# AlgoLab/rs-vgaligner

Hardware: AMD Instinct MI355X
Metric: aligned reads/sec (10 kbp ONT vs HLA graph) (higher is better)
Workload: dtype int32+f64

## Files before the change

### rs-vgaligner_amd/csrc/vga_poa_row.hpp

```cpp
#pragma once

#include "vga_poa_launch.hpp"
#include "vga_poa_kernels.hpp"

#define T4_NEG (4 * POA_NEG)

template <int B>
__device__ __forceinline__ int t4_sub_byte(int a, int g)
{
    int r;
    if constexpr (B == 0) asm("v_sub_u32_sdwa %0, %1, %2 dst_sel:DWORD dst_unused:UNUSED_PAD src0_sel:DWORD src1_sel:BYTE_0" : "=v"(r) : "v"(a), "v"(g));
    if constexpr (B == 1) asm("v_sub_u32_sdwa %0, %1, %2 dst_sel:DWORD dst_unused:UNUSED_PAD src0_sel:DWORD src1_sel:BYTE_1" : "=v"(r) : "v"(a), "v"(g));
    if constexpr (B == 2) asm("v_sub_u32_sdwa %0, %1, %2 dst_sel:DWORD dst_unused:UNUSED_PAD src0_sel:DWORD src1_sel:BYTE_2" : "=v"(r) : "v"(a), "v"(g));
    if constexpr (B == 3) asm("v_sub_u32_sdwa %0, %1, %2 dst_sel:DWORD dst_unused:UNUSED_PAD src0_sel:DWORD src1_sel:BYTE_3" : "=v"(r) : "v"(a), "v"(g));
    return r;
}
template <int B>
__device__ __forceinline__ void t4_gap_byte(int &dst, int &acc, int t, int c)
{
    if constexpr (B == 0) asm("v_min_u32_sdwa %0, %2, %3 dst_sel:BYTE_0 dst_unused:UNUSED_PRESERVE src0_sel:DWORD src1_sel:DWORD\n\tv_cmp_le_u32 vcc, %3, %2\n\tv_addc_co_u32 %1, vcc, %1, %1, vcc" : "+v"(dst), "+v"(acc) : "v"(t), "s"(c) : "vcc");
    if constexpr (B == 1) asm("v_min_u32_sdwa %0, %2, %3 dst_sel:BYTE_1 dst_unused:UNUSED_PRESERVE src0_sel:DWORD src1_sel:DWORD\n\tv_cmp_le_u32 vcc, %3, %2\n\tv_addc_co_u32 %1, vcc, %1, %1, vcc" : "+v"(dst), "+v"(acc) : "v"(t), "s"(c) : "vcc");
    if constexpr (B == 2) asm("v_min_u32_sdwa %0, %2, %3 dst_sel:BYTE_2 dst_unused:UNUSED_PRESERVE src0_sel:DWORD src1_sel:DWORD\n\tv_cmp_le_u32 vcc, %3, %2\n\tv_addc_co_u32 %1, vcc, %1, %1, vcc" : "+v"(dst), "+v"(acc) : "v"(t), "s"(c) : "vcc");
    if constexpr (B == 3) asm("v_min_u32_sdwa %0, %2, %3 dst_sel:BYTE_3 dst_unused:UNUSED_PRESERVE src0_sel:DWORD src1_sel:DWORD\n\tv_cmp_le_u32 vcc, %3, %2\n\tv_addc_co_u32 %1, vcc, %1, %1, vcc" : "+v"(dst), "+v"(acc) : "v"(t), "s"(c) : "vcc");
}
__device__ __forceinline__ void t4_flag_ne(int &acc, int a, int b)
{
    asm("v_cmp_ne_u32 vcc, %1, %2\n\tv_addc_co_u32 %0, vcc, %0, %0, vcc" : "+v"(acc) : "v"(a), "v"(b) : "vcc");
}
template <int B>
__device__ __forceinline__ void t4_flag_ne_dep(int &dst, int acc, int a, int b)
{
    if constexpr (B == 0) asm("v_cmp_ne_u32 vcc, %2, %3\n\tv_addc_co_u32_sdwa %0, vcc, %1, %1, vcc dst_sel:BYTE_0 dst_unused:UNUSED_PRESERVE src0_sel:DWORD src1_sel:DWORD" : "+v"(dst) : "v"(acc), "v"(a), "v"(b) : "vcc");
    if constexpr (B == 1) asm("v_cmp_ne_u32 vcc, %2, %3\n\tv_addc_co_u32_sdwa %0, vcc, %1, %1, vcc dst_sel:BYTE_1 dst_unused:UNUSED_PRESERVE src0_sel:DWORD src1_sel:DWORD" : "+v"(dst) : "v"(acc), "v"(a), "v"(b) : "vcc");
    if constexpr (B == 2) asm("v_cmp_ne_u32 vcc, %2, %3\n\tv_addc_co_u32_sdwa %0, vcc, %1, %1, vcc dst_sel:BYTE_2 dst_unused:UNUSED_PRESERVE src0_sel:DWORD src1_sel:DWORD" : "+v"(dst) : "v"(acc), "v"(a), "v"(b) : "vcc");
    if constexpr (B == 3) asm("v_cmp_ne_u32 vcc, %2, %3\n\tv_addc_co_u32_sdwa %0, vcc, %1, %1, vcc dst_sel:BYTE_3 dst_unused:UNUSED_PRESERVE src0_sel:DWORD src1_sel:DWORD" : "+v"(dst) : "v"(acc), "v"(a), "v"(b) : "vcc");
}
__device__ __forceinline__ int t4_max3(int a, int b, int c)
{
    int r;
    asm("v_max3_i32 %0, %1, %2, %3" : "=v"(r) : "v"(a), "v"(b), "v"(c));
    return r;
}
__device__ __forceinline__ int t4_shr1_max(int v, int pre)
{
    int r = pre;
    asm("s_nop 1\n\tv_max_i32_dpp %0, %1, %2 wave_shr:1 row_mask:0xf bank_mask:0xf" : "+v"(r) : "v"(v), "v"(pre));
    return r;
}
__device__ __forceinline__ int t4_shr1_mov(int v, int first)
{
    int r = first;
    asm("s_nop 1\n\tv_mov_b32_dpp %0, %1 wave_shr:1 row_mask:0xf bank_mask:0xf" : "+v"(r) : "v"(v));
    return r;
}

template <int B>
__device__ __forceinline__ void t5_min_byte(int &dst, int t, int c)
{
    if constexpr (B == 0) asm("v_min_u32_sdwa %0, %1, %2 dst_sel:BYTE_0 dst_unused:UNUSED_PRESERVE src0_sel:DWORD src1_sel:DWORD" : "+v"(dst) : "v"(t), "s"(c));
    if constexpr (B == 1) asm("v_min_u32_sdwa %0, %1, %2 dst_sel:BYTE_1 dst_unused:UNUSED_PRESERVE src0_sel:DWORD src1_sel:DWORD" : "+v"(dst) : "v"(t), "s"(c));
    if constexpr (B == 2) asm("v_min_u32_sdwa %0, %1, %2 dst_sel:BYTE_2 dst_unused:UNUSED_PRESERVE src0_sel:DWORD src1_sel:DWORD" : "+v"(dst) : "v"(t), "s"(c));
    if constexpr (B == 3) asm("v_min_u32_sdwa %0, %1, %2 dst_sel:BYTE_3 dst_unused:UNUSED_PRESERVE src0_sel:DWORD src1_sel:DWORD" : "+v"(dst) : "v"(t), "s"(c));
}

__device__ __forceinline__ int t5_own(int v)
{
    asm volatile("" : "+v"(v));
    return __builtin_amdgcn_readfirstlane(v);
}
__device__ __forceinline__ uint32_t t5_own(uint32_t v) { return (uint32_t)t5_own((int)v); }
__device__ __forceinline__ uint64_t t5_own(uint64_t v) { return ((uint64_t)t5_own((uint32_t)(v >> 32)) << 32) | t5_own((uint32_t)v); }
template <typename T>
__device__ __forceinline__ T *t5_own(T *p) { return (T *)t5_own((uint64_t)p); }


struct poa_row_view {
    int qlen;
    const char *query;
    const uint4 *ntab;
    const uint32_t *plist, *seqw;
    poa_row *R;
    uint32_t n_nodes, ring_rows;
    int bw, banded, p_match, p_mismatch;
};
__device__ __forceinline__ poa_row_view poa_row_view_of(const poa_prob &pb, const char *queries, const uint4 *node_tab, const uint32_t *seq32,
                                                        const uint32_t *preds, const poa_t5_args &A)
{
    poa_row_view V;
    V.qlen = t5_own((int)pb.qlen);
    V.query = queries + pb.q0;
    V.ntab = node_tab + t5_own(pb.node0);
    V.plist = preds + t5_own(pb.pred0);
    V.seqw = seq32 + t5_own(pb.seq0 >> 2);
    V.R = A.rows + t5_own(pb.row0);
    V.n_nodes = t5_own(pb.n_nodes);
    V.ring_rows = t5_own(pb.ring_rows);
    V.bw = t5_own((int)pb.w);
    V.banded = t5_own(A.P.banded);
    V.p_match = t5_own(A.P.match);
    V.p_mismatch = t5_own(A.P.mismatch);
    return V;
}
struct poa_row_pen {
    int o1, e1, o2, e2, D1, D2;
    uint32_t g_bias, e_probe;
};
template <bool DEF>
__device__ __forceinline__ poa_row_pen poa_row_pen_of(const poa_dev_params &P)
{
    poa_row_pen K;
    K.o1 = DEF ? 4 : t5_own(P.o1); K.e1 = DEF ? 2 : t5_own(P.e1); K.o2 = DEF ? 24 : t5_own(P.o2); K.e2 = DEF ? 1 : t5_own(P.e2);
    K.D1 = 4 * K.o1; K.D2 = 4 * K.o2 + 1;
    K.g_bias = (uint32_t)(4 * K.e1 | (4 * K.e2) << 8) * 0x00010001u;
    K.e_probe = (uint32_t)((128 - K.D1) | (128 - K.D2) << 8) * 0x00010001u;
    return K;
}

__device__ __forceinline__ bool poa_row_state(const poa_t5_args &A, int got, bool first_thread, uint64_t &state_lo)
{
    if (got < 0) {
        if (first_thread) {
            poa_out &O = A.outs[blockIdx.x];
            O.t_end = O.t_begin; O.cells = 0; O.vcells = 0; O.maxw = 0; O.nops = 0;
            O.score = POA_NEG; O.row = 0; O.status = A.cp.n_slots ? POA_ST_POOL : POA_ST_RETRY;
        }
        return false;
    }
    __builtin_amdgcn_fence(__ATOMIC_ACQUIRE, "agent");
    state_lo = (uint64_t)A.cp.state_base + (uint64_t)(uint32_t)got * A.cp.state_size;
    return true;
}

struct poa_chunks {
    uint32_t own_head, own_tail, own_chunks;
    uint64_t dcur;
    uint32_t drem;
};
__device__ __forceinline__ uint32_t poa_chunks_pop(const poa_chunk_pool &cp, const poa_chunks &C)
{
    const uint32_t idx = poa_chunk_pop(cp, blockIdx.x);
    if (idx != POA_NIL) __hip_atomic_store(cp.next + idx, C.own_head, __ATOMIC_RELAXED, __HIP_MEMORY_SCOPE_AGENT);
    return idx;
}
__device__ __forceinline__ void poa_chunks_took(poa_chunks &C, uint32_t idx, uint64_t addr)
{
    C.own_head = idx;
    if (C.own_tail == POA_NIL) C.own_tail = idx;
    C.own_chunks++;
    C.dcur = addr;
    C.drem = (uint32_t)POA_CHUNK;
}
__device__ __forceinline__ uint64_t poa_chunks_bump(poa_chunks &C, uint32_t bytes)
{
    const uint64_t r = C.dcur;
    C.dcur += bytes;
    C.drem -= bytes;
    return r;
}

__device__ __forceinline__ int poa_row_codes(uint16_t *Qn, const char *query, int qlen, int n_hw, int tid, int nt)
{
    int non_acgt = 0;
    for (int t = tid; t < n_hw; t += nt) {
        uint32_t hw = 0;
#pragma unroll
        for (int k = 0; k < 4; k++) {
            const int j = 4 * t + k;
            uint32_t code = 0;
            if (j >= 1 && j <= qlen) {
                const char ch = query[j - 1];
                code = (ch == 'A' || ch == 'C' || ch == 'G' || ch == 'T') ? 1u << (((uint32_t)ch >> 1) & 3u) : 0u;
                non_acgt |= code == 0;
            }
            hw |= code << (4 * k);
        }
        Qn[t] = (uint16_t)hw;
    }
    return non_acgt;
}

struct poa_row_topo {
    uint32_t r;
    bool last;
    bool is_sink;
    uint32_t ps;
    uint32_t gb;
    bool simple;
    bool first;
    int np;
    int remain;
};
__device__ __forceinline__ poa_row_topo poa_row_topo_of(const uint4 nt, uint32_t v, uint32_t tn, const uint32_t *seqw, uint32_t &seq_word,
                                                        uint32_t &seq_word_idx)
{
    const uint32_t nlen = nt.y & 0xFFFFFFu;
    const int np_node = (int)(nt.y >> 24);
    poa_row_topo T;
    T.r = nt.x + tn;
    T.last = tn + 1 == nlen;
    T.is_sink = T.last && (nt.z >> 31) != 0;
    T.ps = nt.w;
    T.gb = 0;
    if (v > 0) {
        const uint32_t bi = T.r - 1;
        if ((bi & 3u) == 0 || (bi >> 2) != seq_word_idx) { seq_word_idx = bi >> 2; seq_word = seqw[seq_word_idx]; }
        T.gb = (seq_word >> (8u * (bi & 3u))) & 0xffu;
    }
    T.simple = T.r > 0 && (tn > 0 || (np_node == 1 && T.ps == T.r - 1));
    T.first = tn == 0 && v > 0;
    T.np = v == 0 ? 0 : (tn == 0 ? np_node : 1);
    T.remain = (int)(nt.z & 0x3fffffffu) + (int)(nlen - 1 - tn);
    return T;
}

__device__ __forceinline__ void poa_row_far_span(const poa_row_view &V, const poa_row_topo &T, int prev_lmax, int prev_rmax, int &mpl, int &mpr)
// ... 295 lines not shown
```

### rs-vgaligner_amd/csrc/vga_poa_t5.hpp

```cpp
#pragma once

#include "vga_poa_row.hpp"

__device__ __forceinline__ uint64_t t5_uniform64(uint64_t v)
{
    return ((uint64_t)(uint32_t)__builtin_amdgcn_readfirstlane((int)(v >> 32)) << 32) | (uint32_t)__builtin_amdgcn_readfirstlane((int)(uint32_t)v);
}

#define POA_T5_ARGS_OFFSET 40
__device__ __forceinline__ const poa_t5_args *t5_kargs()
{
    uint32_t off = POA_T5_ARGS_OFFSET;
    asm volatile("" : "+s"(off));
    return (const poa_t5_args *)((const char *)__builtin_amdgcn_kernarg_segment_ptr() + off);
}
template <int NT, bool DEF>
__global__ __launch_bounds__(NT) __attribute__((amdgpu_waves_per_eu(5)))
void k_poa_dp_t5(const poa_prob *__restrict__ probs, const char *__restrict__ queries,
                                                       const uint4 *__restrict__ node_tab, const uint32_t *__restrict__ seq32,
                                                       const uint32_t *__restrict__ preds, const poa_t5_args A)
{
    poa_row *rows = A.rows;
    uint8_t *pool_arg = A.pool;
    const uint32_t lds_cols = t5_own(A.lds_cols), hg_cols = t5_own(A.hg_cols), win_mask = t5_own(A.win_mask);
// ... 144 lines not shown
        }
    }
    if (tid == 0) { sSink[2] = POA_NEG; sSink[3] = 0; }
    int prev_beg = 0, prev_end = -1;
    uint32_t seq_word = 0, seq_word_idx = 0xFFFFFFFFu;

    for (uint32_t v = 0; v < n_nodes && !failed; v++) {
    const uint4 nt = ntab[v];
    const uint32_t nlen = nt.y & 0xFFFFFFu;
    for (uint32_t tn = 0; tn < nlen && !failed; tn++) {
        asm volatile("" : "+s"(st));
        POA_MARK("row_topo");
        const uint32_t r = nt.x + tn;
        const bool last = tn + 1 == nlen;
        const bool is_sink = last && (nt.z >> 31) != 0;
        const uint32_t ps = nt.w;
        uint32_t gb = 0;
        if (v > 0) {
            const uint32_t bi = r - 1;
            if ((bi & 3u) == 0 || (bi >> 2) != seq_word_idx) { seq_word_idx = bi >> 2; seq_word = seqw[seq_word_idx]; }
            gb = (seq_word >> (8u * (bi & 3u))) & 0xffu;
        }
        const bool simple = r > 0 && prev_lds && (tn > 0 || ((nt.y >> 24) == 1u && ps == r - 1));
        const bool writer = wv == (int)(r % (uint32_t)NW);
        POA_MARK("row_prevmax");
        int prev_lmax = 0, prev_rmax = 0;
        if (r > 0) {
            int4 rw = make_int4(INT32_MIN, INT32_MAX, INT32_MIN, 0);
            if (lane < NW) rw = sRed[lane];
            int b = rw.x, t;
            t = poa_dpp<0x111, 0xf>(INT32_MIN, b); b = t > b ? t : b;
            if (NW > 2) { t = poa_dpp<0x112, 0xf>(INT32_MIN, b); b = t > b ? t : b; }
            if (NW > 4) { t = poa_dpp<0x114, 0xf>(INT32_MIN, b); b = t > b ? t : b; }
            if (NW > 8) { t = poa_dpp<0x118, 0xf>(INT32_MIN, b); b = t > b ? t : b; }
            const int rbest = __builtin_amdgcn_readlane(b, NW - 1);
            const uint64_t tie = __builtin_amdgcn_ballot_w64(rw.x == rbest);
            if (__builtin_expect(__builtin_popcountll(tie) == 1, 1)) {
                const int w1 = __builtin_ctzll(tie);
                prev_lmax = __builtin_amdgcn_readlane(rw.y, w1);
                prev_rmax = __builtin_amdgcn_readlane(rw.z, w1);
            } else {
                int lm = rw.x == rbest ? rw.y : INT32_MAX, rm = rw.x == rbest ? rw.z : INT32_MIN;
                t = poa_dpp<0x111, 0xf>(INT32_MAX, lm); lm = t < lm ? t : lm;
                t = poa_dpp<0x111, 0xf>(INT32_MIN, rm); rm = t > rm ? t : rm;
                if (NW > 2) {
                    t = poa_dpp<0x112, 0xf>(INT32_MAX, lm); lm = t < lm ? t : lm;
                    t = poa_dpp<0x112, 0xf>(INT32_MIN, rm); rm = t > rm ? t : rm;
                }
                if (NW > 4) {
                    t = poa_dpp<0x114, 0xf>(INT32_MAX, lm); lm = t < lm ? t : lm;
                    t = poa_dpp<0x114, 0xf>(INT32_MIN, rm); rm = t > rm ? t : rm;
                }
                if (NW > 8) {
                    t = poa_dpp<0x118, 0xf>(INT32_MAX, lm); lm = t < lm ? t : lm;
                    t = poa_dpp<0x118, 0xf>(INT32_MIN, rm); rm = t > rm ? t : rm;
                }
                prev_lmax = __builtin_amdgcn_readlane(lm, NW - 1);
                prev_rmax = __builtin_amdgcn_readlane(rm, NW - 1);
            }
            if (prev_far_use && writer && lane == 0) { R[r - 1].lmax = prev_lmax; R[r - 1].rmax = prev_rmax; }
        }
        POA_MARK("row_setup");
        const int remain = (int)(nt.z & 0x3fffffffu) + (int)(nlen - 1 - tn);
        int beg, end, np, pbeg = prev_beg, pend = prev_end;
        bool first, single, sp_near;
        uint32_t sp = r - 1;
        uint64_t vpo = 0;
        if (__builtin_expect(simple, 1)) {
            first = tn == 0;
            np = 1; single = true; sp_near = true;
            const int mpl = prev_lmax + 1, mpr = prev_rmax + 1;
            if (!P.banded) { beg = 0; end = qlen; }
            else {
                const int diag = qlen - remain;
                const int lo = mpl < diag ? mpl : diag;
                const int hi = mpr > diag ? mpr : diag;
                beg = lo - bw; if (beg < 0) beg = 0;
                end = hi + bw; if (end > qlen) end = qlen;
            }
        } else {
            first = tn == 0 && v > 0;
            np = v == 0 ? 0 : (tn == 0 ? (int)(nt.y >> 24) : 1);
            bool far = r > 0 && !prev_lds;
            if (first) {
                if (np == 1) far |= ps != r - 1;
                else
                    for (int t = 0; t < np; t++) far |= plist[ps + t] != r - 1;
            }
            single = r > 0 && np == 1;
            sp = first ? ps : r - 1;
            sp_near = sp == r - 1 && prev_lds;
            if (far) __syncthreads();
            int mpl, mpr;
            if (r == 0) { mpl = 0; mpr = 0; }
            else if (!first) { mpl = prev_lmax + 1; mpr = prev_rmax + 1; }
            else {
                mpl = INT32_MAX; mpr = 0;
                for (int t = 0; t < np; t++) {
                    const uint32_t p = np == 1 ? ps : plist[ps + t];
                    int lm, rm;
                    if (p == r - 1) { lm = prev_lmax + 1; rm = prev_rmax + 1; }
                    else {
                        lm = __builtin_amdgcn_readfirstlane(R[p].lmax) + 1;
                        rm = __builtin_amdgcn_readfirstlane(R[p].rmax) + 1;
                    }
                    mpl = lm < mpl ? lm : mpl;
                    mpr = rm > mpr ? rm : mpr;
                }
            }
            if (!P.banded) { beg = 0; end = qlen; }
            else {
                const int diag = qlen - remain;
                const int lo = mpl < diag ? mpl : diag;
                const int hi = mpr > diag ? mpr : diag;
                beg = lo - bw; if (beg < 0) beg = 0;
                end = hi + bw; if (end > qlen) end = qlen;
            }
            if (single && !sp_near) {
                pbeg = __builtin_amdgcn_readfirstlane(R[sp].beg);
                pend = __builtin_amdgcn_readfirstlane(R[sp].end);
                vpo = t5_uniform64(R[sp].voff);
            }
        }
        const int bal = beg & ~3;
        const int W = (end - bal + 1 + 3) & ~3;
        const bool wide = (uint32_t)W + 8u > hg_cols;
        const bool keep = last || wide;
        const uint64_t doff = alloc(dcur, dend, (uint32_t)W * (np > 1 ? 4u : 1u), 0);
        uint64_t voff = 0;
        if (last && !failed) {
            if (r == 0 || (nt.z & 0x40000000u)) voff = chunked ? alloc(dcur, dend, 6u * (uint32_t)W, 0) : alloc(vcur, vendp, 6u * (uint32_t)W, 1);
            else {
                voff = ring_base + (uint64_t)ring_head * ((6u * (uint32_t)((qlen + 8) & ~3) + 15u) & ~15u);
                ring_head = ring_head + 1 == ring_rows ? 0 : ring_head + 1;
            }
        } else if (wide) voff = wide_scratch + (r & 1u) * 6ull * lds_cols;
        if (__builtin_expect(failed, 0)) break;
        if (writer && lane == 0) {
            uint32_t *rec = (uint32_t *)(R + r);
            *(uint4 *)rec = make_uint4((uint32_t)beg, (uint32_t)end, (uint32_t)doff, (uint32_t)(doff >> 32));
            *(uint2 *)(rec + 4) = make_uint2((uint32_t)voff, (uint32_t)(voff >> 32));
            *(HIP_vector_type<uint32_t, 3> *)(rec + 8) = HIP_vector_type<uint32_t, 3>(ps, first ? (uint32_t)np : 0u, keep ? 1u : 0u);
        }
        uint8_t *Vrow = pool + voff;
        uint8_t *drow = pool + doff;
        const uint32_t gd = gb - (uint32_t)'A';
        const bool acgt = gd < 20u && ((0x80045u >> gd) & 1u);
        const int sc_eq = acgt ? P.match : 0, sc_ne = acgt ? -P.mismatch : 0;
        const int gsh = (int)((gb >> 1) & 3u);
        const int ne4t = 4 * sc_ne + 1, mm4 = 4 * (sc_eq - sc_ne);
        const bool staged = !simple && r > 0 && !wide && q_plain;
        if (staged) {
            POA_MARK("row_stage");
            if (chunked) {
                bool no_row = false;
                for (int t = 0; t < np; t++) no_row |= t5_uniform64(R[np == 1 ? sp : plist[ps + t]].voff) == 0;
                if (__builtin_expect(no_row, 0)) st |= ST_FAILED;
            }
            for (int c0 = 0; c0 < W; c0 += STEP) {
                const int c = c0 + 4 * tid;
                const int j0 = bal + c;
                if (j0 <= end && np == 1) {
                    const int bp = __builtin_amdgcn_readfirstlane(R[sp].beg), ep = __builtin_amdgcn_readfirstlane(R[sp].end);
                    const uint64_t vq_off = t5_uniform64(R[sp].voff);
                    const uint8_t *Vq = pool + vq_off;
                    const bool vq_ok = !chunked || vq_off != 0;
                    const int balq = bp & ~3;
                    const int Wq = (ep - balq + 1 + 3) & ~3;
                    const int idx = j0 - balq;
                    int4 hv = make_int4(T4_NEG, T4_NEG, T4_NEG, T4_NEG);
                    uint2 gg = make_uint2(0u, 0u);
                    if (idx >= 0 && idx < Wq && vq_ok) {
                        hv = *(const int4 *)((const int32_t *)Vq + idx);
                        gg = *(const uint2 *)(Vq + 4ll * Wq + 2ll * idx);
                    }
                    const unsigned pspan = (unsigned)(ep - bp);
                    const bool in0 = (unsigned)(j0 - bp) <= pspan, in1 = (unsigned)(j0 + 1 - bp) <= pspan, in2 = (unsigned)(j0 + 2 - bp) <= pspan,
                               in3 = (unsigned)(j0 + 3 - bp) <= pspan;
                    hv.x = in0 ? hv.x : T4_NEG; hv.y = in1 ? hv.y : T4_NEG; hv.z = in2 ? hv.z : T4_NEG; hv.w = in3 ? hv.w : T4_NEG;
                    gg.x = (in0 ? gg.x & 0xffffu : 0u) | (in1 ? gg.x & 0xffff0000u : 0u);
                    gg.y = (in2 ? gg.y & 0xffffu : 0u) | (in3 ? gg.y & 0xffff0000u : 0u);
                    *(int4 *)(Hs + (j0 & win_mask)) = hv;
                    *(uint2 *)(Gs + (j0 & win_mask)) = gg;
                    if (c == 0 && bal > 0) {
                        const int wl = (idx >= 1 && idx - 1 < Wq && vq_ok) ? ((const int32_t *)Vq)[idx - 1] : 0;
                        Hs[(bal - 1) & win_mask] = (unsigned)(j0 - 1 - bp) <= pspan ? wl : T4_NEG;
                    }
                } else if (j0 <= end) {
                    int hm[4], x1[4], x2[4], ah[4], a1[4], a2[4];
                    int hl = T4_NEG, ahl = 0;
#pragma unroll
                    for (int k = 0; k < 4; k++) { hm[k] = T4_NEG; x1[k] = T4_NEG; x2[k] = T4_NEG; ah[k] = 0; a1[k] = 0; a2[k] = 0; }
                    for (int t = 0; t < np; t++) {
                        const uint32_t p = np == 1 ? sp : plist[ps + t];
                        const int bp = __builtin_amdgcn_readfirstlane(R[p].beg), ep = __builtin_amdgcn_readfirstlane(R[p].end);
                        const uint64_t vq_off = t5_uniform64(R[p].voff);
                        const uint8_t *Vq = pool + vq_off;
                        const int balq = bp & ~3;
                        const int Wq = (!chunked || vq_off != 0) ? (ep - balq + 1 + 3) & ~3 : 0;
                        const int idx = j0 - balq;
                        int4 hv = make_int4(0, 0, 0, 0);
                        uint2 gg = make_uint2(0u, 0u);
                        if (idx >= 0 && idx < Wq) {
                            hv = *(const int4 *)((const int32_t *)Vq + idx);
                            gg = *(const uint2 *)(Vq + 4ll * Wq + 2ll * idx);
                        }
                        int wl = (idx >= 1 && idx - 1 < Wq) ? ((const int32_t *)Vq)[idx - 1] : 0;
                        const unsigned pspan = (unsigned)(ep - bp);
                        const int hj[4] = {hv.x, hv.y, hv.z, hv.w};
                        const uint32_t g16[4] = {gg.x & 0xffffu, gg.x >> 16, gg.y & 0xffffu, gg.y >> 16};
#pragma unroll
                        for (int k = 0; k < 4; k++) {
                            if ((unsigned)(j0 + k - bp) <= pspan) {
                                const int h = hj[k], c1 = h - (int)(g16[k] & 255u), c2 = h - (int)(g16[k] >> 8);
                                if (h > hm[k]) { hm[k] = h; ah[k] = t; }
                                if (c1 > x1[k]) { x1[k] = c1; a1[k] = t; }
                                if (c2 > x2[k]) { x2[k] = c2; a2[k] = t; }
                            }
                        }
                        if (j0 >= 1 && (unsigned)(j0 - 1 - bp) <= pspan && wl > hl) { hl = wl; ahl = t; }
                    }
                    const int4 hq = make_int4(hm[0], hm[1], hm[2], hm[3]);
                    uint32_t gv[4];
#pragma unroll
                    for (int k = 0; k < 4; k++) gv[k] = (uint32_t)(hm[k] - x1[k]) | ((uint32_t)(hm[k] - x2[k]) << 8);
                    *(int4 *)(Hs + (j0 & win_mask)) = hq;
                    *(uint2 *)(Gs + (j0 & win_mask)) = make_uint2(gv[0] | (gv[1] << 16), gv[2] | (gv[3] << 16));
                    if (c == 0 && bal > 0) Hs[(bal - 1) & win_mask] = hl;
                    if (np > 1) {
                        *(uint32_t *)(drow + (uint64_t)W + c) = (uint32_t)ahl | ((uint32_t)ah[0] << 8) | ((uint32_t)ah[1] << 16) | ((uint32_t)ah[2] << 24);
                        *(uint32_t *)(drow + 2ull * W + c) = (uint32_t)a1[0] | ((uint32_t)a1[1] << 8) | ((uint32_t)a1[2] << 16) | ((uint32_t)a1[3] << 24);
                        *(uint32_t *)(drow + 3ull * W + c) = (uint32_t)a2[0] | ((uint32_t)a2[1] << 8) | ((uint32_t)a2[2] << 16) | ((uint32_t)a2[3] << 24);
                    }
                }
            }
            POA_LDS_BARRIER();
            pbeg = bal > 0 ? bal - 1 : 0;
            pend = bal + W - 1;
        }
        const uint8_t *Vp = pool + vpo;
        const int balp = pbeg & ~3;

        POA_MARK("row_steps");
        enum : uint32_t { F_SINGLE = 1u, F_NEAR = 2u, F_PLAIN = 4u, F_WIDE = 8u, F_KEEP = 16u, F_SINK = 32u, F_MULTI = 64u, F_SRC = 128u };
        const uint32_t rowf = (single ? F_SINGLE : 0u) | (sp_near ? F_NEAR : 0u) | (q_plain ? F_PLAIN : 0u) | (wide ? F_WIDE : 0u) |
                              (keep ? F_KEEP : 0u) | (is_sink ? F_SINK : 0u) | (np > 1 ? F_MULTI : 0u) | (r == 0 ? F_SRC : 0u);
        int best = INT32_MIN, lpos = beg, rpos = beg;
        const bool hot = (simple || staged) && !wide && q_plain;
        const int rlim = end < pend ? end : pend;
        auto run_steps = [&](auto hot_c) __attribute__((always_inline)) {
        constexpr bool HOT = decltype(hot_c)::value;
        int carry1 = POA_IDENT, carry2 = POA_IDENT, left1 = POA_IDENT, left2 = POA_IDENT;
        int next_left = 0;
        int buf = 0;
        for (int c0 = 0; c0 < W; c0 += STEP, buf ^= 1) {
            uint32_t f = HOT ? (rowf & (F_KEEP | F_SINK)) : rowf;
            asm volatile("" : "+s"(f));
            if (HOT) f |= F_SINGLE | F_NEAR | F_PLAIN;
            const int c = c0 + 4 * tid;
            const int j0 = bal + c;
            const bool lane_act = j0 <= end;
            const int jw0 = bal + c0 + 256 * wv, jw1 = jw0 + 255;
            const bool wave_act = jw0 <= end;
            int d_lp = jw0 - beg, d_rp = rlim - jw1, d_lq = (jw0 > beg ? jw0 : beg) - pbeg - 1;
            asm volatile("" : "+s"(d_lp), "+s"(d_rp), "+s"(d_lq));
            const uint32_t e_lp = (uint32_t)d_lp >> 31;
            const uint32_t e_rp = (uint32_t)d_rp >> 31;
            const uint32_t e_lq = (uint32_t)d_lq >> 31;
            const bool lp = e_lp != 0, rp = e_rp != 0, lq = e_lq != 0;
            int htt[4], ht4[4], e1t[4], e2t[4], pmeta[4];
            int agg1 = POA_IDENT, agg2 = POA_IDENT, alast1 = POA_IDENT, alast2 = POA_IDENT;
#pragma unroll
            for (int k = 0; k < 4; k++) { htt[k] = T4_NEG + 2; ht4[k] = T4_NEG; e1t[k] = T4_NEG + 1; e2t[k] = T4_NEG; pmeta[k] = 0; }
            uint32_t qn = 0u;
            if (wave_act) qn = (uint32_t)Qn[j0 >> 2];
            const bool fastw = HOT ? wave_act
                                   : (f & (F_SINGLE | F_PLAIN)) == (F_SINGLE | F_PLAIN) && wave_act && (!lq || (f & F_NEAR)) && (!rp || ((f & F_NEAR) && end <= pend + 1));
            const int base1 = 4 * e1 * j0, base2 = 4 * e2 * j0;
        if constexpr (HOT) POA_MARK("hot_p1_fast"); else POA_MARK("p1_fast");
            if (__builtin_expect(fastw, 1)) {
                int4 hv;
                uint2 gg;
                int hprev;
                if constexpr (HOT) {
                    hv = *(const int4 *)(Hs + (j0 & win_mask));
                    gg = *(const uint2 *)(Gs + (j0 & win_mask));
                    int left0;
                    if (wv == 0 && c0 > 0) left0 = next_left;
                    else left0 = Hs[(jw0 > 0 ? jw0 - 1 : 0) & (int)win_mask];
                    if (wv == 0 && c0 + STEP < W) next_left = Hs[(jw0 + STEP - 1) & (int)win_mask];
                    hprev = t4_shr1_mov(hv.w, left0);
                } else if (__builtin_expect((f & F_NEAR) != 0, 1)) {
                    hv = *(const int4 *)(Hs + (j0 & win_mask));
                    gg = *(const uint2 *)(Gs + (j0 & win_mask));
                    if (tid == NT - 1) edgeW[buf] = hv.w;
                    {
                        const bool edge = tid == 0 && c0 > 0;
                        int w = Hs[edge ? edge_idx + (buf ^ 1) : ((j0 > 0 ? j0 - 1 : 0) & win_mask)];
                        asm volatile("" : "+v"(w));
                        hprev = w;
                    }
                } else {
                    const int Wp = (pend - balp + 1 + 3) & ~3;
                    const int idx = j0 - balp;
                    hv = *(const int4 *)((const int32_t *)Vp + idx);
                    gg = *(const uint2 *)(Vp + 4ll * Wp + 2ll * idx);
                    hprev = ((const int32_t *)Vp)[idx > 0 ? idx - 1 : 0];
                    asm volatile("" : "+v"(hv.x), "+v"(hv.y), "+v"(hv.z), "+v"(hv.w), "+v"(gg.x), "+v"(gg.y), "+v"(hprev));
                }
                auto phase1 = [&](auto edge_c) {
                    constexpr bool EDGE = decltype(edge_c)::value;
                    int hj[4] = {hv.x, hv.y, hv.z, hv.w};
                    int ga = (int)gg.x, gbb = (int)gg.y;
                    if constexpr (EDGE) {
                        if (rp) {
#pragma unroll
                            for (int k = 0; k < 4; k++) hj[k] = j0 + k > pend ? T4_NEG : hj[k];
                            ga = j0 > pend ? 0 : (j0 + 1 > pend ? (ga & 0xffff) : ga);
                            gbb = j0 + 2 > pend ? 0 : (j0 + 3 > pend ? (gbb & 0xffff) : gbb);
                        }
                        if (lq) {
#pragma unroll
                            for (int k = 0; k < 4; k++) hj[k] = j0 + k < pbeg ? T4_NEG : hj[k];
                            ga = j0 + 1 < pbeg ? 0 : (j0 < pbeg ? (int)((uint32_t)ga & 0xffff0000u) : ga);
                            gbb = j0 + 3 < pbeg ? 0 : (j0 + 2 < pbeg ? (int)((uint32_t)gbb & 0xffff0000u) : gbb);
                        }
                    }
                    const uint32_t eqb = qn >> gsh;
                    int hp = hprev;
                    if constexpr (EDGE && HOT) {
                        if (rp) hp = j0 - 1 > pend ? T4_NEG : hp;
                    }
#pragma unroll
                    for (int k = 0; k < 4; k++) {
                        const int g = k < 2 ? ga : gbb;
                        const int ev1 = (k & 1) ? t4_sub_byte<2>(hj[k], g) : t4_sub_byte<0>(hj[k], g);
                        const int ev2 = (k & 1) ? t4_sub_byte<3>(hj[k], g) : t4_sub_byte<1>(hj[k], g);
                        int m = (int)__umul24(__builtin_amdgcn_ubfe(eqb, 4u * k, 1u), (uint32_t)mm4) + (hp + ne4t);
                        if constexpr (EDGE) {
                            if (lq) m = j0 + k - 1 < pbeg ? T4_NEG + 2 : m;
                        }
                        const int h = t4_max3(m, ev1, ev2);
                        htt[k] = h;
                        ht4[k] = h & ~3;
                        e1t[k] = ev1;
                        e2t[k] = ev2;
                        hp = hj[k];
                    }
                    if constexpr (EDGE) {
                        if (lp) {
#pragma unroll
                            for (int k = 0; k < 4; k++) ht4[k] = j0 + k < beg ? POA_IDENT : ht4[k];
                        }
                    }
                    const int r11 = ht4[1] + 4 * e1, r12 = ht4[2] + 8 * e1, r13 = ht4[3] + 12 * e1;
                    const int r21 = ht4[1] + 4 * e2, r22 = ht4[2] + 8 * e2, r23 = ht4[3] + 12 * e2;
                    const int a1 = t4_max3(ht4[0], r11, r12), a2 = t4_max3(ht4[0], r21, r22);
                    agg1 = (a1 > r13 ? a1 : r13) + base1;
                    agg2 = (a2 > r23 ? a2 : r23) + base2;
                    alast1 = r13 + base1;
                    alast2 = r23 + base2;
                };
                if (__builtin_expect((e_lp | e_rp | e_lq) != 0, 0)) phase1(std::true_type{});
                else phase1(std::false_type{});
        if constexpr (HOT) POA_MARK("hot_p1_lean"); else POA_MARK("p1_lean");
            } else if (wave_act && (f & F_SINGLE)) {
                int pbeg_ = pbeg, pend_ = pend, beg_ = beg, end_ = end, balp_ = balp, gsh_ = gsh;
                asm volatile("" : "+s"(pbeg_), "+s"(pend_), "+s"(beg_), "+s"(end_), "+s"(balp_), "+s"(gsh_));
                const int pbeg = pbeg_, pend = pend_, beg = beg_, end = end_, balp = balp_, gsh = gsh_;
                const unsigned span = (unsigned)(end - beg), pspan = (unsigned)(pend - pbeg);
                int hj[4], wm0;
                uint32_t g16[4];
                if (f & F_NEAR) {
                    const int4 hv = *(const int4 *)(Hs + (j0 & win_mask));
                    const uint2 gg = *(const uint2 *)(Gs + (j0 & win_mask));
                    hj[0] = hv.x; hj[1] = hv.y; hj[2] = hv.z; hj[3] = hv.w;
                    g16[0] = gg.x & 0xffffu; g16[1] = gg.x >> 16; g16[2] = gg.y & 0xffffu; g16[3] = gg.y >> 16;
                    if (tid == NT - 1) edgeW[buf] = hj[3];
                    const bool edge = tid == 0 && c0 > 0;
                    int w = Hs[edge ? edge_idx + (buf ^ 1) : ((j0 > 0 ? j0 - 1 : 0) & win_mask)];
                    asm volatile("" : "+v"(w));
                    wm0 = w;
                } else {
                    const int idx = j0 - balp;
                    const int Wp = (pend - balp + 1 + 3) & ~3;
                    int4 hv = make_int4(0, 0, 0, 0);
                    uint2 gg = make_uint2(0u, 0u);
// ... 390 lines not shown
```

Baseline: 10630.

## Merge two-predecessor rows from LDS window instead of reloading from global pool

Adds a staged path for rows with exactly two predecessors where one is the immediately previous row. That predecessor's H and gap values are read from the LDS window instead of the global pool, and they are merged with the far predecessor using packed SDWA compare/flag instructions to build the traceback bytes. Columns are walked in reverse with a barrier so in-place LDS overwrites are safe. The general path also hoists predecessor metadata loads out of the per-column loop. The cost is added code complexity, an extra barrier per column step, and more register pressure.

```diff
diff --git a/rs-vgaligner_amd/csrc/vga_poa_row.hpp b/rs-vgaligner_amd/csrc/vga_poa_row.hpp
--- a/rs-vgaligner_amd/csrc/vga_poa_row.hpp
+++ b/rs-vgaligner_amd/csrc/vga_poa_row.hpp
@@ -61,6 +61,15 @@
     if constexpr (B == 1) asm("v_min_u32_sdwa %0, %1, %2 dst_sel:BYTE_1 dst_unused:UNUSED_PRESERVE src0_sel:DWORD src1_sel:DWORD" : "+v"(dst) : "v"(t), "s"(c));
     if constexpr (B == 2) asm("v_min_u32_sdwa %0, %1, %2 dst_sel:BYTE_2 dst_unused:UNUSED_PRESERVE src0_sel:DWORD src1_sel:DWORD" : "+v"(dst) : "v"(t), "s"(c));
     if constexpr (B == 3) asm("v_min_u32_sdwa %0, %1, %2 dst_sel:BYTE_3 dst_unused:UNUSED_PRESERVE src0_sel:DWORD src1_sel:DWORD" : "+v"(dst) : "v"(t), "s"(c));
+}
+
+template <int B>
+__device__ __forceinline__ void t5_flag_gt_byte(int &dst, int a, int b, int zero)
+{
+    if constexpr (B == 0) asm("v_cmp_gt_i32 vcc, %2, %3\n\tv_addc_co_u32_sdwa %0, vcc, %1, %1, vcc dst_sel:BYTE_0 dst_unused:UNUSED_PRESERVE src0_sel:DWORD src1_sel:DWORD" : "+v"(dst) : "v"(zero), "v"(a), "v"(b) : "vcc");
+    if constexpr (B == 1) asm("v_cmp_gt_i32 vcc, %2, %3\n\tv_addc_co_u32_sdwa %0, vcc, %1, %1, vcc dst_sel:BYTE_1 dst_unused:UNUSED_PRESERVE src0_sel:DWORD src1_sel:DWORD" : "+v"(dst) : "v"(zero), "v"(a), "v"(b) : "vcc");
+    if constexpr (B == 2) asm("v_cmp_gt_i32 vcc, %2, %3\n\tv_addc_co_u32_sdwa %0, vcc, %1, %1, vcc dst_sel:BYTE_2 dst_unused:UNUSED_PRESERVE src0_sel:DWORD src1_sel:DWORD" : "+v"(dst) : "v"(zero), "v"(a), "v"(b) : "vcc");
+    if constexpr (B == 3) asm("v_cmp_gt_i32 vcc, %2, %3\n\tv_addc_co_u32_sdwa %0, vcc, %1, %1, vcc dst_sel:BYTE_3 dst_unused:UNUSED_PRESERVE src0_sel:DWORD src1_sel:DWORD" : "+v"(dst) : "v"(zero), "v"(a), "v"(b) : "vcc");
 }
 
 __device__ __forceinline__ int t5_own(int v)
diff --git a/rs-vgaligner_amd/csrc/vga_poa_t5.hpp b/rs-vgaligner_amd/csrc/vga_poa_t5.hpp
--- a/rs-vgaligner_amd/csrc/vga_poa_t5.hpp
+++ b/rs-vgaligner_amd/csrc/vga_poa_t5.hpp
@@ -320,17 +320,114 @@
         const bool staged = !simple && r > 0 && !wide && q_plain;
         if (staged) {
             POA_MARK("row_stage");
+            uint32_t p0 = 0, p1 = 0;
+            if (np > 1) { p0 = plist[ps]; p1 = plist[ps + 1]; }
+            const bool lds_join = np == 2 && prev_lds && p0 != p1 && (p0 == r - 1 || p1 == r - 1);
+            if (lds_join) {
+                POA_MARK("row_stage_lds");
+                const bool near_second = p1 == r - 1;
+                const uint32_t pf = near_second ? p0 : p1;
+                int fb = R[pf].beg, fe = R[pf].end;
+                uint64_t fv = R[pf].voff;
+                if (__builtin_expect(chunked && t5_uniform64(fv) == 0, 0)) st |= ST_FAILED;
+                int nb = prev_beg;
+                unsigned nspan = (unsigned)(prev_end - prev_beg);
+                asm volatile("" : "+v"(nb), "+v"(nspan), "+v"(fb), "+v"(fe), "+v"(fv));
+                const int fbv = fb;
+                const unsigned fspan = (unsigned)(fe - fb);
+                const uint8_t *Vq = pool + fv;
+                const int balq = fb & ~3;
+                const int Wq = (!chunked || fv != 0) ? (fe - balq + 1 + 3) & ~3 : 0;
+                for (int c0 = (W - 1) & ~(STEP - 1); c0 >= 0; c0 -= STEP) {
+                    const int c = c0 + 4 * tid;
+                    const int j0 = bal + c;
+                    const bool act = j0 <= end;
+                    int4 hn = make_int4(0, 0, 0, 0), hf = make_int4(0, 0, 0, 0);
+                    uint2 gn = make_uint2(0u, 0u), gf = make_uint2(0u, 0u);
+                    int wn = 0, wf = 0;
+                    if (act) {
+                        const int idx = j0 - balq;
+                        if (idx >= 0 && idx < Wq) {
+                            hf = *(const int4 *)((const int32_t *)Vq + idx);
+                            gf = *(const uint2 *)(Vq + 4ll * Wq + 2ll * idx);
+                        }
+                        if (idx >= 1 && idx - 1 < Wq) wf = ((const int32_t *)Vq)[idx - 1];
+                        hn = *(const int4 *)(Hs + (j0 & win_mask));
+                        gn = *(const uint2 *)(Gs + (j0 & win_mask));
+                        wn = Hs[(j0 > 0 ? j0 - 1 : 0) & win_mask];
+                    }
+                    POA_LDS_BARRIER();
+                    if (act) {
+                        auto mask_band = [&](int4 &hv, uint2 &gg, int &wl, int bp, unsigned pspan) {
+                            if (!((unsigned)(j0 - 1 - bp) <= pspan && (unsigned)(j0 + 3 - bp) <= pspan)) {
+                                const bool in0 = (unsigned)(j0 - bp) <= pspan, in1 = (unsigned)(j0 + 1 - bp) <= pspan,
+                                           in2 = (unsigned)(j0 + 2 - bp) <= pspan, in3 = (unsigned)(j0 + 3 - bp) <= pspan;
+                                hv.x = in0 ? hv.x : T4_NEG; hv.y = in1 ? hv.y : T4_NEG; hv.z = in2 ? hv.z : T4_NEG; hv.w = in3 ? hv.w : T4_NEG;
+                                gg.x = (in0 ? gg.x & 0xffffu : 0u) | (in1 ? gg.x & 0xffff0000u : 0u);
+                                gg.y = (in2 ? gg.y & 0xffffu : 0u) | (in3 ? gg.y & 0xffff0000u : 0u);
+                                wl = (j0 >= 1 && (unsigned)(j0 - 1 - bp) <= pspan) ? wl : T4_NEG;
+                            }
+                        };
+                        mask_band(hn, gn, wn, nb, nspan);
+                        mask_band(hf, gf, wf, fbv, fspan);
+                        auto merge = [&](const int4 &ha, const uint2 &ga, int wa, const int4 &hb, const uint2 &gb2, int wb) {
+                            const int A[4] = {ha.x, ha.y, ha.z, ha.w}, B[4] = {hb.x, hb.y, hb.z, hb.w};
+                            int zero = 0;
+                            asm volatile("" : "+v"(zero));
+                            int ph = 0, pa1 = 0, pa2 = 0;
+                            int hm[4];
+                            uint32_t gv[4];
+                            const int tl = wa > T4_NEG ? wa : T4_NEG;
+                            const int hl = wb > tl ? wb : tl;
+                            t5_flag_gt_byte<0>(ph, wb, tl, zero);
+#pragma unroll
+                            for (int k = 0; k < 4; k++) {
+                                const int g_a = (int)(k < 2 ? ga.x : ga.y), g_b = (int)(k < 2 ? gb2.x : gb2.y);
+                                const int ca1 = (k & 1) ? t4_sub_byte<2>(A[k], g_a) : t4_sub_byte<0>(A[k], g_a);
+                                const int ca2 = (k & 1) ? t4_sub_byte<3>(A[k], g_a) : t4_sub_byte<1>(A[k], g_a);
+                                const int cb1 = (k & 1) ? t4_sub_byte<2>(B[k], g_b) : t4_sub_byte<0>(B[k], g_b);
+                                const int cb2 = (k & 1) ? t4_sub_byte<3>(B[k], g_b) : t4_sub_byte<1>(B[k], g_b);
+                                const int th = A[k] > T4_NEG ? A[k] : T4_NEG, t1 = ca1 > T4_NEG ? ca1 : T4_NEG, t2 = ca2 > T4_NEG ? ca2 : T4_NEG;
+                                hm[k] = B[k] > th ? B[k] : th;
+                                const int x1 = cb1 > t1 ? cb1 : t1, x2 = cb2 > t2 ? cb2 : t2;
+                                if (k == 0) { t5_flag_gt_byte<1>(ph, B[k], th, zero); t5_flag_gt_byte<0>(pa1, cb1, t1, zero); t5_flag_gt_byte<0>(pa2, cb2, t2, zero); }
+                                if (k == 1) { t5_flag_gt_byte<2>(ph, B[k], th, zero); t5_flag_gt_byte<1>(pa1, cb1, t1, zero); t5_flag_gt_byte<1>(pa2, cb2, t2, zero); }
+                                if (k == 2) { t5_flag_gt_byte<3>(ph, B[k], th, zero); t5_flag_gt_byte<2>(pa1, cb1, t1, zero); t5_flag_gt_byte<2>(pa2, cb2, t2, zero); }
+                                if (k == 3) { t5_flag_gt_byte<3>(pa1, cb1, t1, zero); t5_flag_gt_byte<3>(pa2, cb2, t2, zero); }
+                                gv[k] = (uint32_t)(hm[k] - x1) | ((uint32_t)(hm[k] - x2) << 8);
+                            }
+                            *(int4 *)(Hs + (j0 & win_mask)) = make_int4(hm[0], hm[1], hm[2], hm[3]);
+                            *(uint2 *)(Gs + (j0 & win_mask)) = make_uint2(gv[0] | (gv[1] << 16), gv[2] | (gv[3] << 16));
+                            if (c == 0 && bal > 0) Hs[(bal - 1) & win_mask] = hl;
+                            *(uint32_t *)(drow + (uint64_t)W + c) = (uint32_t)ph;
+                            *(uint32_t *)(drow + 2ull * W + c) = (uint32_t)pa1;
+                            *(uint32_t *)(drow + 3ull * W + c) = (uint32_t)pa2;
+                        };
+                        if (near_second) merge(hf, gf, wf, hn, gn, wn);
+                        else merge(hn, gn, wn, hf, gf, wf);
+                    }
+                }
+            } else {
+            POA_MARK("row_stage_far");
+            int qb0 = pbeg, qe0 = pend, qb1 = 0, qe1 = -1;
+            uint64_t qv0 = vpo, qv1 = 0;
+            if (np > 1) {
+                qb0 = R[p0].beg; qe0 = R[p0].end; qv0 = R[p0].voff;
+                qb1 = R[p1].beg; qe1 = R[p1].end; qv1 = R[p1].voff;
+            }
             if (chunked) {
-                bool no_row = false;
-                for (int t = 0; t < np; t++) no_row |= t5_uniform64(R[np == 1 ? sp : plist[ps + t]].voff) == 0;
+                bool no_row = np >= 1 && t5_uniform64(qv0) == 0;
+                if (np > 1) no_row |= t5_uniform64(qv1) == 0;
+                for (int t = 2; t < np; t++) no_row |= t5_uniform64(R[plist[ps + t]].voff) == 0;
                 if (__builtin_expect(no_row, 0)) st |= ST_FAILED;
             }
+            asm volatile("" : "+v"(qb0), "+v"(qe0), "+v"(qv0), "+v"(qb1), "+v"(qe1), "+v"(qv1));
             for (int c0 = 0; c0 < W; c0 += STEP) {
                 const int c = c0 + 4 * tid;
                 const int j0 = bal + c;
                 if (j0 <= end && np == 1) {
-                    const int bp = __builtin_amdgcn_readfirstlane(R[sp].beg), ep = __builtin_amdgcn_readfirstlane(R[sp].end);
-                    const uint64_t vq_off = t5_uniform64(R[sp].voff);
+                    const int bp = qb0, ep = qe0;
+                    const uint64_t vq_off = qv0;
                     const uint8_t *Vq = pool + vq_off;
                     const bool vq_ok = !chunked || vq_off != 0;
                     const int balq = bp & ~3;
@@ -360,9 +457,12 @@
 #pragma unroll
                     for (int k = 0; k < 4; k++) { hm[k] = T4_NEG; x1[k] = T4_NEG; x2[k] = T4_NEG; ah[k] = 0; a1[k] = 0; a2[k] = 0; }
                     for (int t = 0; t < np; t++) {
-                        const uint32_t p = np == 1 ? sp : plist[ps + t];
-                        const int bp = __builtin_amdgcn_readfirstlane(R[p].beg), ep = __builtin_amdgcn_readfirstlane(R[p].end);
-                        const uint64_t vq_off = t5_uniform64(R[p].voff);
+                        int bp = t == 0 ? qb0 : qb1, ep = t == 0 ? qe0 : qe1;
+                        uint64_t vq_off = t == 0 ? qv0 : qv1;
+                        if (t >= 2) {
+                            const uint32_t p = plist[ps + t];
+                            bp = R[p].beg; ep = R[p].end; vq_off = R[p].voff;
+                        }
                         const uint8_t *Vq = pool + vq_off;
                         const int balq = bp & ~3;
                         const int Wq = (!chunked || vq_off != 0) ? (ep - balq + 1 + 3) & ~3 : 0;
@@ -401,6 +501,7 @@
                         *(uint32_t *)(drow + 3ull * W + c) = (uint32_t)a2[0] | ((uint32_t)a2[1] << 8) | ((uint32_t)a2[2] << 16) | ((uint32_t)a2[3] << 24);
                     }
                 }
+            }
             }
             POA_LDS_BARRIER();
             pbeg = bal > 0 ? bal - 1 : 0;
```

Result: no change. 10670, median of 3 (+0.4%).
